# blubs/OpenGLRaytracer

Measured on AMD Instinct MI355X. Metric: primary Mrays/s at 1920×1080; achieved HBM GB/s vs peak; 1/2/4/8-GPU scaling, higher is better.
Workload: dtype f32

## Files before the change

include/rt.h:

```cpp
#ifndef OPENGLRAYTRACER_AMD_RT_H
#define OPENGLRAYTRACER_AMD_RT_H

#include <stddef.h>
#include <stdint.h>

#ifdef __cplusplus
extern "C" {
#endif

#define RT_OK 0
#define RT_ERR_INVALID (-1)
#define RT_ERR_HIP (-2)
#define RT_ERR_NOMEM (-3)
#define RT_ERR_UNSUPPORTED (-4)
#define RT_ERR_NO_DEVICE (-5)

#define RT_MAX_DEPTH 9

typedef struct rt_material {
    float ambient[4];
    float diffuse[4];
    float specular[4];
    float shininess;
    float emissive[4];
// ... 132 lines not shown

typedef struct rt_multi rt_multi;
#define RT_MULTI_RCCL 0
#define RT_MULTI_COPY 1
int rt_multi_create(int n_gpus, rt_context *const *ctxs, int transport, rt_multi **out);
void rt_multi_destroy(rt_multi *m);
int rt_render_multi(rt_multi *m, const rt_scene *const *scenes, const rt_camera *cam, float time, int width,
                    int height, int max_depth, int block_rows, float *out, int out_is_device);
int rt_render_multi_view(rt_multi *m, const rt_scene *const *scenes, const rt_view *view, int width, int height,
                         int max_depth, int block_rows, float *out, int out_is_device);
int rt_multi_last_ms(rt_multi *m, float *kernel_ms, float *gather_ms, float *assemble_ms);

#define RT_OPT_CULLING 1
#define RT_OPT_TIMING 2
#define RT_OPT_OUTPUT 3
#define RT_OUTPUT_RGBA32F 0
#define RT_OUTPUT_RGBA8 1
#define RT_OUTPUT_RGB32F 2
#define RT_OPT_FRAME_CONSTS 4
#define RT_OPT_ORIGIN_LISTS 7
#define RT_OPT_SCENE_SHAPES 8
#define RT_OPT_LAUNCH_SHAPES 9
#define RT_OPT_PERSISTENT0 10
int rt_context_set(rt_context *ctx, int option, int value);

int rt_last_kernel_ms(rt_context *ctx, float *ms);

int rt_pack_rgba8(const float *rgba32f, size_t n_pixels, uint8_t *out_rgba8);

int rt_write_ppm(const char *path, const float *rgba32f, int width, int height);
int rt_write_pfm(const char *path, const float *rgba32f, int width, int height);

const char *rt_last_error(void);
const char *rt_version(void);

#ifdef __cplusplus
}
#endif
#endif
```

openglraytracer_amd/__init__.py:

```python
import ctypes as C
import os

import numpy as np

from .abi import (RT_MAX_DEPTH, RT_OK, Camera, Light, Material, Object)
from . import abi

_HERE = os.path.dirname(os.path.abspath(__file__))
LIB_PATH = os.path.join(_HERE, "libopenglraytracer_amd.so")
_lib = None


class RTError(RuntimeError):
    def __init__(self, code, msg):
        super().__init__("rt error %d: %s" % (code, msg))
        self.code = code


class View(C.Structure):
    _fields_ = [("unprojection", C.c_float * 16), ("origin", C.c_float * 3)]


def lib():
    global _lib
# ... 218 lines not shown
        return self._h

    def set_culling(self, on):
        _check(lib().rt_context_set(self._h, abi.RT_OPT_CULLING, 1 if on else 0))

    def set_timing(self, on):
        _check(lib().rt_context_set(self._h, abi.RT_OPT_TIMING, 1 if on else 0))

    def set_host_frame_consts(self, on):
        _check(lib().rt_context_set(self._h, abi.RT_OPT_FRAME_CONSTS, 1 if on else 0))

    def set_origin_lists(self, on):
        _check(lib().rt_context_set(self._h, abi.RT_OPT_ORIGIN_LISTS, 1 if on else 0))

    def set_scene_shapes(self, on):
        _check(lib().rt_context_set(self._h, abi.RT_OPT_SCENE_SHAPES, 1 if on else 0))

    def set_launch_shapes(self, on):
        _check(lib().rt_context_set(self._h, abi.RT_OPT_LAUNCH_SHAPES, 1 if on else 0))

    def set_persistent0(self, value):
        _check(lib().rt_context_set(self._h, abi.RT_OPT_PERSISTENT0, int(value)))

    def set_output(self, fmt):
        _check(lib().rt_context_set(self._h, abi.RT_OPT_OUTPUT, fmt))
        self.output = fmt

    def last_kernel_ms(self):
        ms = C.c_float()
        _check(lib().rt_last_kernel_ms(self._h, C.byref(ms)))
        return ms.value


class Scene:

    def __init__(self, ctx, objects, materials=None, lights=None):
        materials = materials if materials is not None else reference_materials()
        lights = lights if lights is not None else reference_lights()
        objs = (Object * max(len(objects), 1))(*objects)
        mats = (Material * len(materials))(*materials)
        lts = (Light * max(len(lights), 1))(*lights)
        self._h = C.c_void_p()
        _check(lib().rt_scene_create(ctx.handle, objs, len(objects), mats, len(materials), lts,
                                     len(lights), C.byref(self._h)))
        self.ctx = ctx

# ... 219 lines not shown
```

openglraytracer_amd/abi.py:

```python
import ctypes as C

import numpy as np

RT_OK = 0
RT_ERR_INVALID = -1
RT_ERR_HIP = -2
RT_ERR_NOMEM = -3
RT_ERR_UNSUPPORTED = -4
RT_ERR_NO_DEVICE = -5
RT_MAX_DEPTH = 9
RT_MAX_OBJECTS = 1024
RT_MAX_LIGHTS = 16
RT_MAX_MATERIALS = 256
RT_OPT_CULLING = 1
RT_OPT_TIMING = 2
RT_OPT_OUTPUT = 3
RT_OPT_FRAME_CONSTS = 4
RT_OPT_ORIGIN_LISTS = 7
RT_OPT_SCENE_SHAPES = 8
RT_OPT_LAUNCH_SHAPES = 9
RT_OPT_PERSISTENT0 = 10
RT_OUTPUT_RGBA32F = 0
RT_OUTPUT_RGBA8 = 1
RT_OUTPUT_RGB32F = 2
RT_MAX_BATCH = 256
RT_MULTI_RCCL = 0
RT_MULTI_COPY = 1
RT_ANIM_NONE = 0
RT_ANIM_RATE = 1
RT_ANIM_RATE_OFFSET = 2
RT_ANIM_SIN = 3
RT_ANIM_SIN_OFFSET = 4

MATERIAL1, MATERIAL2, RED_GLASS, GREEN_GLASS, BLUE_GLASS, MIRROR, WALL = range(7)
MATERIAL_NAMES = ["material1", "material2", "red_glass_material", "green_glass_material",
                  "blue_glass_material", "mirror_material", "wall_material"]

F3 = C.c_float * 3
F4 = C.c_float * 4


class Material(C.Structure):
    _fields_ = [("ambient", F4), ("diffuse", F4), ("specular", F4), ("shininess", C.c_float),
                ("emissive", F4), ("reflectivity", C.c_float), ("transparency", C.c_float),
# ... 37 lines not shown
```

openglraytracer_amd/csrc/rt_api.cpp:

```cpp
#include <hip/hip_runtime.h>

#include <algorithm>
#include <climits>
#include <cmath>
#include <cstdio>
#include <cstring>
#include <new>
#include <string>
#include <type_traits>
#include <vector>

#include "build_id.h"
#include "rt_anim.h"
#include "rt_internal.h"

namespace rtamd {

namespace {
thread_local std::string g_error;
}

void set_error(const std::string &msg) { g_error = msg; }

int hip_fail(const char *what, hipError_t e) {
// ... 20 lines not shown
        set_error("null context or scene");
        return RT_ERR_INVALID;
    }
    if (scene->device != ctx->device) {
        set_error("scene was created on another device");
        return RT_ERR_INVALID;
    }
    if (width <= 0 || height <= 0 || width > 65536 || height > 65536) {
        set_error("bad frame size");
        return RT_ERR_INVALID;
    }
    if (max_depth < 0 || max_depth > RT_MAX_DEPTH) {
        set_error("max_depth " + std::to_string(max_depth) + " outside [0, " + std::to_string(RT_MAX_DEPTH) + "]");
        return RT_ERR_UNSUPPORTED;
    }
    return RT_OK;
}

bool fill_view(const rt_context *ctx, const rt_view &view, int width, int height, FrameView &v) {
    v = FrameView{};
    v.cull = (view_projection(view, v.proj) && ctx->culling) ? 1 : 0;
    std::memcpy(v.unproj, view.unprojection, sizeof v.unproj);
    std::memcpy(v.origin, view.origin, sizeof v.origin);
    return camera_short_divisions(v.unproj, width, height);
}

LaunchParams base_params(const rt_context *ctx, const rt_scene *scene, const rt_view *views, int n_views,
                         int width, int height, LaunchHost &h) {
    LaunchParams p{};
    p.n_views = n_views;
    p.cam_short = 1;
    h = LaunchHost{};
    h.shape_cull = ctx->scene_shapes;
    h.shape_launch = ctx->launch_shapes;
    h.persistent0 = ctx->persistent0;
    h.n_cu = ctx->n_cu;
    for (int k = 0; k < n_views; ++k) {
        if (!fill_view(ctx, views[k], width, height, p.view[k])) p.cam_short = 0;
        if (!p.view[k].cull) h.shape_cull = 0;
    }
    p.width = width;
    p.height = height;
    const DeviceScene &d = scene->dev;
    h.scene_room = d.room;
    p.scene = d.blob;
    p.layout = d.layout;
    if (!ctx->origin_lists) p.layout.off_olist = -1;
    p.out_format = ctx->output;
    if (ctx->host_consts) {
        const float4 *blobs[kMaxViews];
        for (int k = 0; k < n_views; ++k) blobs[k] = scene->host.empty() ? nullptr : scene->host.data();
        host_frame_setup(p, blobs);
    }
    return p;
}

int launch(rt_context *ctx, LaunchParams &p, const LaunchHost &h, int max_depth, hipStream_t stream) {
    const unsigned slot = ctx->sched_next % kSchedSlots;
// ... 187 lines not shown
        h.shape_cull = f[21];
        p.layout.off_dmask = f[22] > 0 ? 0 : -1;
        p.layout.dmask_bytes = f[22];
        p.layout.dmask_n = kShapeMaskTexels;
    }
    h.shape_launch = f[1];
    p.width = f[2];
    p.height = f[3];
    p.row_begin = f[4];
    p.n_rows = f[5];
    p.block_rows = f[6];
    p.n_shards = f[7];
    p.shard = f[8];
    p.out_format = f[9];
    p.n_frame_consts = f[10];
    p.cam_short = f[11];
    p.slice_begin = f[12];
    p.slice_rows = f[13];
    p.spp = f[14];
    return launch_shape(p, h, f[0], resident);
}
int rt_debug_launch_shape(const int32_t *f) { return rt_debug_launch_shape_n(f, 15); }
int rt_debug_last_queued(const rt_context *ctx) { return ctx ? (ctx->last_queued ? 1 : 0) : RT_ERR_INVALID; }
int rt_debug_last_scene_shape(const rt_context *ctx) { return ctx ? ctx->last_shape : RT_ERR_INVALID; }
int rt_debug_persistent_chunk(int c, int total, int waves, int32_t *out) {
    if (!out || c < 0 || total < 0 || total >= (1 << 30) || waves <= 0) return RT_ERR_INVALID;
    const ChunkRange r = persistent_chunk(c, total, waves);
    out[0] = r.t;
    out[1] = r.t_end;
    return RT_OK;
}
int rt_debug_persistent_queue(int g, int waves, int32_t *out) {
    if (!out || g < 0 || waves <= 0 || g >= waves) return RT_ERR_INVALID;
    out[0] = persistent_queue(g);
    out[1] = persistent_queue_waves(out[0], waves);
    out[2] = persistent_first_chunk(g);
    return RT_OK;
}
const char *rt_version(void) { return "openglraytracer_amd 0.3 (gfx950, " RT_BUILD_ID ")"; }

int rt_create(int device, rt_context **out) {
    if (!out) { set_error("rt_create: null out"); return RT_ERR_INVALID; }
    *out = nullptr;
    int n = 0;
    hipError_t e = hipGetDeviceCount(&n);
    if (e != hipSuccess || n <= 0) {
        set_error("rt_create: no HIP device");
// ... 472 lines not shown
    LaunchHost h;
    LaunchParams p = base_params(ctx, scene, view, 1, width, height, h);
    p.row_begin = row_begin;
    p.n_rows = row_end - row_begin;
    p.spp = spp;
    p.sample0 = sample_offset;
    p.seed = seed;
    p.jitter = jitter ? 1 : 0;
    p.out = reinterpret_cast<float4 *>(accum_device);
    hipStream_t stream = hip_stream ? static_cast<hipStream_t>(hip_stream) : ctx->stream;
    if ((rc = launch_scene(ctx, scene, p, h, max_depth, stream)) != RT_OK) return rc;
    return finish_call(hip_stream, stream);
}

int rt_context_set(rt_context *ctx, int option, int value) {
    if (!ctx) { set_error("rt_context_set: null context"); return RT_ERR_INVALID; }
    switch (option) {
        case RT_OPT_CULLING: ctx->culling = value ? 1 : 0; return RT_OK;
        case RT_OPT_TIMING: ctx->timing = value ? 1 : 0; return RT_OK;
        case RT_OPT_FRAME_CONSTS: ctx->host_consts = value ? 1 : 0; return RT_OK;
        case RT_OPT_ORIGIN_LISTS: ctx->origin_lists = value ? 1 : 0; return RT_OK;
        case RT_OPT_SCENE_SHAPES: ctx->scene_shapes = value ? 1 : 0; return RT_OK;
        case RT_OPT_LAUNCH_SHAPES: ctx->launch_shapes = value ? 1 : 0; return RT_OK;
        case RT_OPT_PERSISTENT0:
            if (value < 0 || (value > 1 && value < 8)) {
                set_error("rt_context_set: RT_OPT_PERSISTENT0 takes 0, 1 or a work-group cap of at least 8");
                return RT_ERR_INVALID;
            }
            ctx->persistent0 = value;
            return RT_OK;
        case RT_OPT_OUTPUT:
            if (value != RT_OUTPUT_RGBA32F && value != RT_OUTPUT_RGBA8 && value != RT_OUTPUT_RGB32F) {
                set_error("rt_context_set: unknown output format " + std::to_string(value));
                return RT_ERR_INVALID;
            }
            ctx->output = value;
            return RT_OK;
        default: set_error("rt_context_set: unknown option " + std::to_string(option)); return RT_ERR_INVALID;
    }
}

int rt_last_kernel_ms(rt_context *ctx, float *ms) {
    if (!ctx || !ms || !ctx->timed) {
        set_error("rt_last_kernel_ms: nothing timed yet");
        return RT_ERR_INVALID;
    }
// ... 256 lines not shown
```

openglraytracer_amd/csrc/rt_internal.h:

```cpp
#pragma once

#include <hip/hip_runtime.h>

#include <cstddef>
#include <cstdint>
#include <memory>
#include <string>
#include <vector>

#include "../../include/rt.h"

namespace rtamd {

struct SphereRec {
    float cx, cy, cz, rr;
};
struct SphereMeta {
    int32_t obj_index;
    int32_t material;
    float radius;
    int32_t pad;
};

struct BoxRec {
// ... 49 lines not shown
#define RT_OLIST_FROM 33
#endif
constexpr int kOListMinSpheres = RT_OLIST_FROM;
constexpr float kOListBoundUnit = 1.0f / 256.0f;
struct BvhNode {
    float lo[3];
    int32_t skip;
    float hi[3];
    int32_t leaf;
};
static_assert(sizeof(BvhNode) == 32, "BvhNode layout");
constexpr int kBvhOctants = 8;

struct LightRec {
    float pos[3];
    float dead;
};

struct FrameView {
    float unproj[16];
    float proj[16];
    float origin[3];
    int32_t cull;
    const void *blob;
};
constexpr int kMaxViews = 8;
constexpr int kBatchSlots = 4;
constexpr int kMaxFrameConsts = 272;
constexpr int kMaxViewConsts = 256;
constexpr size_t kMaxLds = 160 * 1024;

struct SceneLayout {
    int32_t off_spheres, off_smeta, off_boxes, off_mats, off_lights, off_lightmat;
    int32_t off_bvh, n_bvh;
    int32_t off_blink;
    int32_t off_cone;
    int32_t off_dmask, dmask_n;
    int32_t dmask_bytes;
    int32_t off_gmask, gmask_words;
    int32_t off_glist;
    int32_t blob_units;
    int32_t off_olist;
    int32_t dmask_box;
    int32_t off_bplane;
    int32_t n_spheres, n_boxes, n_mats, n_lights;
};

struct LaunchParams {
    FrameView view[kMaxViews];
    int32_t n_views;
    int32_t width, height;
    int32_t row_begin, n_rows;
    int32_t block_rows, n_shards, shard;
    const void *scene;
    float4 *out;
    int32_t spp, sample0, jitter;
    uint32_t seed;
    SceneLayout layout;
    int32_t *sched;
    int32_t out_format;
    int32_t n_frame_consts;
    int32_t cam_short;
    int32_t slice_begin, slice_rows;
    const FrameView *views_dev;
    const float4 *consts_dev;
    float4 frame_consts[kMaxFrameConsts];
};
static_assert(sizeof(LaunchParams) == 5776, "kernel argument block: the hidden arguments' offsets");
static_assert(offsetof(LaunchParams, layout) % 16 == 0, "the layout's offsets: aligned scalar loads (see above)");
static_assert(offsetof(LaunchParams, frame_consts) + sizeof(LaunchParams::frame_consts) == sizeof(LaunchParams),
              "kernarg_probe reads the last record: nothing the kernels read lies behind it");
static_assert(sizeof(LaunchParams) <= 6144, "kernel argument block");
struct LaunchHost {
    int32_t shape_cull;
    int32_t scene_room;
    int32_t shape_launch;
    int32_t persistent0;
    int32_t n_cu;
};
constexpr int kShapeMaskBytes = 15;
constexpr int kShapeMaskTexels = 12;
constexpr int kShapeRoom = 16;
constexpr int kShapeWide = 32;
int scene_shape(const SceneLayout &L, const LaunchHost &h, int max_depth);
constexpr int kLaunchPlain = 1;
constexpr int kLaunchPersistent = 2;
int launch_shape(const LaunchParams &p, const LaunchHost &h, int max_depth, int resident = 0);
#ifndef RT_CHUNK0
#define RT_CHUNK0 16
#endif
constexpr int kChunk0 = RT_CHUNK0;
static_assert(kChunk0 >= 2 && kChunk0 <= 32 && (kChunk0 & (kChunk0 - 1)) == 0, "bulk chunk: a power of two, 2..32");
struct ChunkRange {
    int t, t_end;
};
__host__ __device__ inline ChunkRange persistent_chunk(int c, int total, int waves) {
    int start = 0;
#pragma unroll
    for (int s = kChunk0; s >= 2; s >>= 1) {
        const int left = (total - start) / s - waves;
        const int n = left > 0 ? left : 0;
        if (c < n) return {start + c * s, start + c * s + s};
        c -= n;
        start += n * s;
    }
    return c < total - start ? ChunkRange{start + c, start + c + 1} : ChunkRange{total, total};
// ... 58 lines not shown
int ensure_origin_lists(rt_context *ctx, const rt_scene *scene, int max_depth);
int note_scene_use(const rt_scene *scene, hipStream_t stream, std::shared_ptr<UseEvent> *shared = nullptr);
int launch_scene(rt_context *ctx, const rt_scene *scene, LaunchParams &p, const LaunchHost &h, int max_depth,
                 hipStream_t stream);
inline size_t surface_bytes(int fmt) { return fmt == RT_OUTPUT_RGBA8 ? 4 : (fmt == RT_OUTPUT_RGB32F ? 12 : 16); }

}

struct rt_context {
    int device = 0;
    hipStream_t stream = nullptr;
    hipEvent_t ev0 = nullptr, ev1 = nullptr;
    float4 *staging = nullptr;
    size_t staging_px = 0;
    bool timed = false;
    int culling = 1;
    int timing = 1;
    int output = RT_OUTPUT_RGBA32F;
    int host_consts = 1;
    int origin_lists = 1;
    int scene_shapes = 1;
    int launch_shapes = 1;
    int persistent0 = 1;
    void *batch_dev[rtamd::kBatchSlots] = {};
    void *batch_host[rtamd::kBatchSlots] = {};
    hipEvent_t batch_done[rtamd::kBatchSlots] = {};
    bool batch_used[rtamd::kBatchSlots] = {};
    unsigned batch_next = 0;
    int n_cu = 0;
    int32_t *sched = nullptr;
    unsigned sched_next = 0;
    hipEvent_t sched_done[rtamd::kSchedSlots] = {};
    bool sched_used[rtamd::kSchedSlots] = {};
    bool last_queued = false;
    int last_shape = 0;
    std::vector<struct rt_scene *> scenes;
};

struct rt_scene {
    int device = 0;
    rtamd::DeviceScene dev;
    std::vector<float4> host;
    int32_t capacity_units = 0;
    rt_context *ctx = nullptr;
    static constexpr int kMaxUseStreams = 8;
    using Event = rtamd::UseEvent;
// ... 9 lines not shown
```

openglraytracer_amd/csrc/rt_kernel.hip:

```cpp
#include <hip/hip_runtime.h>

#include <algorithm>
#include <climits>
#include <cstdint>
#include <string>

#include "rt_internal.h"

namespace rtamd {
namespace {

constexpr int kWavesX = 2, kWavesY = 2;
constexpr int kTileX = 8 * kWavesX, kTileY = 8 * kWavesY;
constexpr int kThreads = 64 * kWavesX * kWavesY;

struct v3 {
    float x, y, z;
};
__device__ __forceinline__ v3 mk(float x, float y, float z) { return {x, y, z}; }
__device__ __forceinline__ v3 add(v3 a, v3 b) { return {a.x + b.x, a.y + b.y, a.z + b.z}; }
__device__ __forceinline__ v3 sub(v3 a, v3 b) { return {a.x - b.x, a.y - b.y, a.z - b.z}; }
__device__ __forceinline__ v3 muls(v3 a, float s) { return {a.x * s, a.y * s, a.z * s}; }
__device__ __forceinline__ v3 sel(bool c, v3 a, v3 b) { return {c ? a.x : b.x, c ? a.y : b.y, c ? a.z : b.z}; }
__device__ __forceinline__ float dot(v3 a, v3 b) { return a.x * b.x + (a.y * b.y + a.z * b.z); }

#ifdef RT_FAST_MATH
#define RT_FAST_DIV
#define RT_FAST_RSQ
// ... 1309 lines not shown
__device__ __forceinline__ Pixel wave_pixel(const LaunchParams &p, int wx, int wy) {
    const int lane = threadIdx.x & 63;
    Pixel px;
    px.x = wx * 8 + (lane & 7);
    if constexpr ((kLaunch & kLaunchPlain) != 0) {
        px.local_row = wy * 8 + (lane >> 3);
        px.active = px.x < p.width && px.local_row < p.height;
        px.y = px.active ? px.local_row : wy * 8;
        return px;
    }
    px.local_row = p.slice_begin + wy * 8 + (lane >> 3);
    px.active = px.x < p.width && px.local_row < p.slice_begin + p.slice_rows;
    px.y = output_row(p, px.active ? px.local_row : p.slice_begin + wy * 8);
    return px;
}

template <int kLaunch = 0>
__device__ __forceinline__ Ray camera_ray(const LaunchParams &p, const FrameView &V, int x, int y, float jx,
                                          float jy) {
    constexpr bool kPlain = (kLaunch & kLaunchPlain) != 0;
    const int hw = p.width / 2, hh = p.height / 2;
    const float *M = V.unproj;
    const float nx = static_cast<float>(x - hw) + jx, ny = static_cast<float>(y - hh) + jy;
    float vx, vy;
    if (kPlain || (hw > 0 && hh > 0)) {
        vx = div_r(nx, rcp_refined(static_cast<float>(hw)));
        vy = div_r(ny, rcp_refined(static_cast<float>(hh)));
    } else {
        vx = nx / static_cast<float>(hw);
        vy = ny / static_cast<float>(hh);
    }
    float ws[4], we[4];
#pragma unroll
    for (int k = 0; k < 4; ++k) {
        ws[k] = M[k] * vx + M[4 + k] * vy + M[8 + k] * 0.5f + M[12 + k] * 1.0f;
        we[k] = M[k] * vx + M[4 + k] * vy + M[8 + k] * 1.0f + M[12 + k] * 1.0f;
    }
    v3 s3, e3;
    if (kPlain || p.cam_short) {
        const Rcp rs3 = rcp_refined(ws[3]), re3 = rcp_refined(we[3]);
        s3 = mk(div_r(ws[0], rs3), div_r(ws[1], rs3), div_r(ws[2], rs3));
        e3 = mk(div_r(we[0], re3), div_r(we[1], re3), div_r(we[2], re3));
    } else {
        s3 = mk(fdiv(ws[0], ws[3]), fdiv(ws[1], ws[3]), fdiv(ws[2], ws[3]));
        e3 = mk(fdiv(we[0], we[3]), fdiv(we[1], we[3]), fdiv(we[2], we[3]));
    }
    Ray ray;
    ray.start = mk(V.origin[0], V.origin[1], V.origin[2]);
    ray.dir = normalize(sub(e3, s3));
    return ray;
}


template <int kDepth, bool kAccum, int kShape, int kLaunch = 0>
__device__ __forceinline__ void render_wave_tile(const LaunchParams &p, Scene S, const FrameView &V, int wx, int wy,
                                                 int z, const Pixel &px, const Ray &pre, bool have_pre) {
    S.cull = V.cull;
    S.room = 0;
// ... 91 lines not shown
    asm volatile("" : "+s"(a));
    return *(const LaunchParams *)a;
}
__device__ __forceinline__ float4 *persistent_slot(const LaunchParams &p, float4 *lds) {
    return lds + p.layout.blob_units + __builtin_amdgcn_readfirstlane(threadIdx.x >> 6) * p.n_frame_consts;
}
__device__ __forceinline__ void persistent_refill(const LaunchParams &p, float4 *lds, int z) {
    float4 *const slot = persistent_slot(p, lds);
    RT_PHASE_CLOCK(refill_t0);
    __builtin_amdgcn_fence(__ATOMIC_RELEASE, "wavefront");
    __builtin_amdgcn_wave_barrier();
    int lane = threadIdx.x & 63;
    asm volatile("" : "+v"(lane));
    for (int i = lane; i < p.n_frame_consts; i += 64) slot[i] = p.consts_dev[z * p.n_frame_consts + i];
    __builtin_amdgcn_fence(__ATOMIC_ACQUIRE, "wavefront");
    __builtin_amdgcn_wave_barrier();
    RT_PHASE_SPAN(10, 12, refill_t0);
}
template <int kShape, int kLaunch>
__device__ __forceinline__ void persistent_tile(const LaunchParams &p, float4 *lds, int z, int wx, int wy) {
    const float4 *blob = static_cast<const float4 *>(p.scene);
    float4 *const slot = persistent_slot(p, lds);
    const SceneLayout &L = p.layout;
    Scene S;
    S.sph = lds + L.off_spheres;
    S.smeta = reinterpret_cast<const int4 *>(lds + L.off_smeta);
    S.sph_cam = slot;
    S.sph_px = reinterpret_cast<const int4 *>(slot + L.n_spheres);
    S.box = reinterpret_cast<const BoxRec *>(lds + L.off_boxes);
    S.box_cam = slot + 2 * L.n_spheres;
    S.mat = reinterpret_cast<const MatRec *>(lds + L.off_mats);
    S.light = reinterpret_cast<const LightRec *>(lds + L.off_lights);
    S.lm = reinterpret_cast<const LightMatRec *>(lds + L.off_lightmat);
    S.bvh = lds + L.off_bvh;
    S.blink = reinterpret_cast<const uint32_t *>(lds + L.off_blink);
    S.cone = nullptr;
    S.dmask = reinterpret_cast<const char *>(lds + L.off_dmask);
    S.dmask_n = kShapeMaskTexels;
    S.dmask_bytes = kShape & kShapeMaskBytes;
    S.dmask_box = L.dmask_box;
    S.cbplane = L.off_bplane >= 0 ? (const __attribute__((address_space(4))) float4 *)(blob + L.off_bplane) : nullptr;
    S.gmask = nullptr;
    S.gwords = 0;
    S.glist = nullptr;
    S.olist = nullptr;
    S.cbox = (const __attribute__((address_space(4))) BoxRec *)(blob + L.off_boxes);
    S.clight = (const __attribute__((address_space(4))) LightRec *)(blob + L.off_lights);
#ifdef RT_UNIFORM_MAT
    S.cmat = (const __attribute__((address_space(4))) MatRec *)(blob + L.off_mats);
    S.clm = (const __attribute__((address_space(4))) LightMatRec *)(blob + L.off_lightmat);
#endif
    S.nbvh = 0;
    S.ns = L.n_spheres;
    S.nb = L.n_boxes;
    S.nl = L.n_lights;
    S.nm = L.n_mats;
    const FrameView V = cload((const __attribute__((address_space(4))) FrameView *)(p.views_dev) + z);
    const Ray none{mk(0.0f, 0.0f, 0.0f), mk(0.0f, 0.0f, 0.0f)};
    render_wave_tile<0, false, kShape, kLaunch>(p, S, V, wx, wy, z, wave_pixel<kLaunch>(p, wx, wy), none, false);
}
template <int kShape, int kLaunch>
__device__ __forceinline__ void render_persistent0(float4 *lds) {
    static_assert((kLaunch & kLaunchPlain) != 0 && (kShape & kShapeMaskBytes) != 0, "plain shaped launches");
    __builtin_amdgcn_s_setprio(1);
    RT_PHASE(0);
#ifdef RT_PHASE_TRACE
    if (RT_PHASE_LANE0) {
        RT_PHASE_SLOT(8) = __builtin_amdgcn_s_getreg((31 << 11) | 4) | (unsigned long long)__builtin_amdgcn_s_getreg((31 << 11) | 20) << 32;
    }
#endif
    {
        const LaunchParams &p = launch_args();
        const float4 *blob = static_cast<const float4 *>(p.scene);
// ... 273 lines not shown
    const void *fn = reinterpret_cast<const void *>(&render_kernel<kDepth, kAccum, kDev, kShape, kLaunch>);
    dim3 grid((p.width + kTileX - 1) / kTileX, (p.slice_rows + kTileY - 1) / kTileY, p.n_views);
    const int wave_tiles = ((p.width + 7) / 8) * ((p.slice_rows + 7) / 8) * p.n_views;
    const int resident = h.n_cu > 0 ? groups_per_cu(fn, lds) * h.n_cu : 0;
    bool one_scene = p.n_views <= kMaxViews;
    for (int k = 0; k < p.n_views && one_scene; ++k) one_scene = p.view[k].blob == nullptr;
    if (kQueuedDepth(kDepth) && p.sched && wave_tiles > resident * (kThreads / 64) &&
        resident * (kThreads / 64) >= kQueues &&
        (p.n_views == 1 || (one_scene && queued_views_for(fn, p.layout, kLean) >= p.n_views))) {
        grid = dim3(resident, 1, 1);
        lds = queued_lds_bytes(p.layout, kLean, p.n_views);
    } else {
        p.sched = nullptr;
    }
    hipLaunchKernelGGL((render_kernel<kDepth, kAccum, kDev, kShape, kLaunch>), grid, dim3(kThreads), lds, stream, p);
    return hipGetLastError();
}

size_t persistent_lds_bytes(const LaunchParams &p) {
    return (static_cast<size_t>(p.layout.blob_units) + static_cast<size_t>(kThreads / 64) * p.n_frame_consts) * sizeof(float4);
}

template <bool kAccum, bool kDev, int kShape>
hipError_t launch_shaped0(LaunchParams &p, const LaunchHost &h, hipStream_t stream) {
    if constexpr (!kAccum) {
        if ((launch_shape(p, h, 0) & kLaunchPlain) != 0) {
            if constexpr (kDev) {
                constexpr int kPersistent = kLaunchPlain | kLaunchPersistent;
                const size_t lds = persistent_lds_bytes(p);
                if (h.persistent0 > 0 && p.sched && lds <= kMaxLds && h.n_cu > 0) {
                    const void *fn = reinterpret_cast<const void *>(&render_kernel<0, false, true, kShape, kPersistent>);
                    const int groups = persistent_groups(p, h, groups_per_cu(fn, lds) * h.n_cu);
                    if (groups > 0) {
                        hipLaunchKernelGGL((render_kernel<0, false, true, kShape, kPersistent>), dim3(groups),
                                           dim3(kThreads), lds, stream, p);
                        return hipGetLastError();
                    }
                }
            }
            return launch_kernel<0, false, kDev, kShape, kLaunchPlain>(p, h, stream);
        }
    }
    return launch_kernel<0, kAccum, kDev, kShape>(p, h, stream);
}
template <bool kAccum, bool kDev>
hipError_t launch_depth0(LaunchParams &p, const LaunchHost &h, hipStream_t stream) {
    switch (scene_shape(p.layout, h, 0)) {
        case 2: return launch_shaped0<kAccum, kDev, 2>(p, h, stream);
        case 4: return launch_shaped0<kAccum, kDev, 4>(p, h, stream);
        case 8: return launch_shaped0<kAccum, kDev, 8>(p, h, stream);
        case 2 | kShapeRoom: return launch_shaped0<kAccum, kDev, 2 | kShapeRoom>(p, h, stream);
        case 4 | kShapeRoom: return launch_shaped0<kAccum, kDev, 4 | kShapeRoom>(p, h, stream);
        case 8 | kShapeRoom: return launch_shaped0<kAccum, kDev, 8 | kShapeRoom>(p, h, stream);
        default: return launch_kernel<0, kAccum, kDev, 0>(p, h, stream);
    }
}

template <int kDepth>
hipError_t launch_deep(LaunchParams &p, const LaunchHost &h, hipStream_t stream) {
    switch (scene_shape(p.layout, h, kDepth)) {
        case kShapeWide: return launch_kernel<kDepth, false, false, kShapeWide>(p, h, stream);
        case kShapeWide | kShapeRoom: return launch_kernel<kDepth, false, false, kShapeWide | kShapeRoom>(p, h, stream);
        default: return launch_kernel<kDepth, false, false, 0>(p, h, stream);
    }
}

template <int kDepth>
hipError_t launch_depth(LaunchParams &p, const LaunchHost &h, hipStream_t stream) {
    if (p.views_dev) {
        if constexpr (kDepth == 0) {
            if (p.spp == 0) return launch_depth0<false, true>(p, h, stream);
        } else if constexpr (kDepth == 1) {
            if (p.spp == 0) return launch_kernel<kDepth, false, true>(p, h, stream);
        }
        return hipErrorInvalidValue;
    }
    if constexpr (kDepth == 0) return p.spp > 0 ? launch_depth0<true, false>(p, h, stream) : launch_depth0<false, false>(p, h, stream);
    if constexpr (kDepth >= 2) {
        if (p.spp == 0) return launch_deep<kDepth>(p, h, stream);
    }
    return p.spp > 0 ? launch_kernel<kDepth, true>(p, h, stream) : launch_kernel<kDepth, false>(p, h, stream);
}

}

int scene_shape(const SceneLayout &L, const LaunchHost &h, int max_depth) {
    if (!h.shape_cull) return 0;
    const int box = L.n_boxes == 1 && h.scene_room ? kShapeRoom : 0;
    if (max_depth == 0) {
        if (L.off_dmask < 0 || (L.dmask_bytes != 2 && L.dmask_bytes != 4 && L.dmask_bytes != 8) ||
            L.dmask_n != kShapeMaskTexels)
            return 0;
        return L.dmask_bytes | box;
    }
    if (max_depth >= 2) {
        if (L.off_gmask < 0 || L.off_glist < 0 || L.off_olist < 0) return 0;
        return kShapeWide | box;
    }
    return 0;
}

int persistent_groups(const LaunchParams &p, const LaunchHost &h, int resident) {
#if defined(RT_STATS) || defined(RT_CYCLES)
    return 0;
#endif
    if (h.persistent0 <= 0 || (launch_shape(p, h, 0) & kLaunchPlain) == 0 || scene_shape(p.layout, h, 0) == 0) return 0;
    if (!p.views_dev || !p.consts_dev || p.n_views <= kMaxViews || !p.sched) return 0;
    const bool forced = h.persistent0 >= 8;
    const int groups = forced && h.persistent0 < resident ? h.persistent0 : resident;
    const long long waves = static_cast<long long>(groups) * (kThreads / 64);
    const long long tiles = static_cast<long long>((p.width + 7) / 8) * ((p.height + 7) / 8) * p.n_views;
    if (waves < kQueues || tiles >= (1ll << 30)) return 0;
    if (!forced && tiles < kPersistentMinTilesPerWave * waves) return 0;
    return groups;
}

// ... 74 lines not shown
        (void)hipFree(d);
    }
    if (e != hipSuccess) {
        set_error(std::string("rt_create: kernel argument probe: ") + hipGetErrorString(e));
        return RT_ERR_HIP;
    }
    if (h[0].x != 1.5f || h[0].y != -2.25f || h[0].z != 3.125f || h[0].w != 4096.0f ||
        __builtin_bit_cast(uint32_t, h[1].x) != 0x5a5au || __builtin_bit_cast(uint32_t, h[1].y) != 0x3c3cu) {
        set_error("rt_create: this HIP runtime does not pass a " + std::to_string(sizeof(LaunchParams)) +
                  "-byte kernel argument block intact");
        return RT_ERR_UNSUPPORTED;
    }
    return RT_OK;
}

hipError_t allow_large_lds(size_t bytes) {
#define RT_KFN(d) reinterpret_cast<const void *>(&render_kernel<d, false>), \
                  reinterpret_cast<const void *>(&render_kernel<d, true>)
#define RT_SHAPES(k) reinterpret_cast<const void *>(&render_kernel<0, false, false, k>), \
                     reinterpret_cast<const void *>(&render_kernel<0, true, false, k>),  \
                     reinterpret_cast<const void *>(&render_kernel<0, false, true, k>),  \
                     reinterpret_cast<const void *>(&render_kernel<0, false, false, k, kLaunchPlain>), \
                     reinterpret_cast<const void *>(&render_kernel<0, false, true, k, kLaunchPlain>), \
                     reinterpret_cast<const void *>(&render_kernel<0, false, true, k, kLaunchPlain | kLaunchPersistent>)
#define RT_WIDE(d) reinterpret_cast<const void *>(&render_kernel<d, false, false, kShapeWide>), \
                   reinterpret_cast<const void *>(&render_kernel<d, false, false, kShapeWide | kShapeRoom>)
    const void *fns[] = {RT_KFN(0), RT_KFN(1), RT_KFN(2), RT_KFN(3), RT_KFN(4),
                         RT_KFN(5), RT_KFN(6), RT_KFN(7), RT_KFN(8), RT_KFN(9),
                         reinterpret_cast<const void *>(&render_kernel<0, false, true>),
                         reinterpret_cast<const void *>(&render_kernel<1, false, true>),
                         RT_SHAPES(2), RT_SHAPES(4), RT_SHAPES(8),
                         RT_SHAPES(2 | kShapeRoom), RT_SHAPES(4 | kShapeRoom), RT_SHAPES(8 | kShapeRoom),
                         RT_WIDE(2), RT_WIDE(3), RT_WIDE(4), RT_WIDE(5), RT_WIDE(6), RT_WIDE(7), RT_WIDE(8), RT_WIDE(9)};
#undef RT_KFN
#undef RT_SHAPES
#undef RT_WIDE
    for (const void *f : fns)
        (void)hipFuncSetAttribute(f, hipFuncAttributeMaxDynamicSharedMemorySize, static_cast<int>(bytes));
    (void)hipGetLastError();
    return hipSuccess;
}

}

#ifdef RT_STATS
extern "C" int rt_debug_stats(unsigned long long *dst, int clear) {
    if (hipMemcpyFromSymbol(dst, HIP_SYMBOL(rtamd::rt_stats), sizeof(rtamd::rt_stats), 0, hipMemcpyDeviceToHost) !=
// ... 42 lines not shown
```

openglraytracer_amd/csrc/rt_scene.cpp:

```cpp
#include <algorithm>
#include <cmath>
#include <cstring>
#include <map>
#include <memory>
#include <mutex>
#include <new>
#include <system_error>
#include <thread>
#include <vector>

#include "rt_anim.h"
#include "rt_internal.h"

using namespace rtamd;

namespace {

constexpr float kPi = 3.14159265358f;
constexpr float kDegToRad = kPi / 180.0f;

struct M4 {
    double m[4][4];
};

// ... 1011 lines not shown
        for (int i = 0; i < n_objs; ++i)
            for (int k = 0; k < 3; ++k)
                finite = finite && std::isfinite(objs[i].position[k]) && std::isfinite(objs[i].box_mins[k]) &&
                         std::isfinite(objs[i].box_maxs[k]) && std::isfinite(objs[i].radius);
        bplane.assign(boxes.size() * static_cast<size_t>(n_lights), no_plane());
        for (size_t b = 0; b < boxes.size() && finite; ++b)
            for (int j = 0; j < n_lights; ++j)
                bplane[b * n_lights + j] = box_light_plane(boxes[b], lights[j].position, extent);
        lay.off_bplane = off;
        off += units(bplane.size() * sizeof(float4));
    }
    lay.off_bvh = off;     off += units(bvh.size() * sizeof(BvhNode));
    lay.off_blink = off;   off += units(blink.size() * sizeof(uint32_t));
    const size_t per_frame = sph.size() * 32 + boxes.size() * 16;
    int n_live = 0;
    for (int j = 0; j < n_lights; ++j) n_live += lrec[j].dead == 0.0f;
    std::vector<uint64_t> dmask;
    lay.off_dmask = -1;
    lay.dmask_n = 0;
    const bool box_bits = boxes.size() >= 2;
    const size_t mask_bits = sph.size() + (box_bits ? boxes.size() : 0);
    lay.dmask_box = 0;
    lay.dmask_bytes = 4;
    if (!sph.empty() && mask_bits <= static_cast<size_t>(kMaskMaxSpheres) && n_live > 0) {
        lay.dmask_bytes = mask_bits <= 16 ? 2 : (mask_bits <= 32 ? 4 : 8);
#ifndef RT_DMASK_MAXN
#define RT_DMASK_MAXN 12
#endif
        for (int n : {32, 24, 16, 12, 8}) {
            if (n > RT_DMASK_MAXN) continue;
            const size_t bytes = static_cast<size_t>(n_live) * 6 * n * n * lay.dmask_bytes;
            if ((static_cast<size_t>(off) + units(bytes)) * 16 + per_frame <= kMaskLdsBudget) {
                lay.dmask_n = n;
                break;
            }
        }
    }
    std::vector<char> dmask_bytes;
    if (lay.dmask_n > 0) {
        if (box_bits) {
            std::vector<SphereRec> bsph(sph);
            std::vector<SphereMeta> bmeta(smeta);
            for (size_t b = 0; b < boxes.size(); ++b) {
                bsph.push_back({ball[b].x, ball[b].y, ball[b].z, 0.0f});
                bmeta.push_back({boxes[b].obj_index, boxes[b].material, ball[b].w, 0});
            }
            build_direction_masks(bsph, bmeta, lights, lrec, lay.dmask_n, dmask);
            lay.dmask_box = 1;
        } else {
            build_direction_masks(sph, smeta, lights, lrec, lay.dmask_n, dmask);
        }
        lay.off_dmask = off;
        dmask_bytes.resize(dmask.size() * lay.dmask_bytes);
        for (size_t i = 0; i < dmask.size(); ++i)
            std::memcpy(dmask_bytes.data() + i * lay.dmask_bytes, &dmask[i], lay.dmask_bytes);
        off += units(dmask_bytes.size());
        cones.clear();
    }
    const size_t with_cones = (static_cast<size_t>(off) + units(cones.size() * sizeof(ShadowCone))) * 16 + per_frame;
    if (lay.dmask_n == 0 && with_cones <= kConeLdsBudget) {
        lay.off_cone = off;
        off += units(cones.size() * sizeof(ShadowCone));
    } else {
        lay.off_cone = -1;
        cones.clear();
    }
    lay.n_bvh = static_cast<int32_t>(bvh.size());
    lay.blob_units = off;
    std::vector<uint64_t> gmask;
    std::vector<uint8_t> glist;
    lay.off_gmask = -1;
    lay.off_glist = -1;
    lay.gmask_words = 0;
#ifndef RT_GMASK_FROM
#define RT_GMASK_FROM 32
#endif
    if (sph.size() > static_cast<size_t>(RT_GMASK_FROM) &&
        sph.size() <= static_cast<size_t>(kGMaskMaxSpheres) && n_live > 0) {
        lay.gmask_words = static_cast<int32_t>((sph.size() + 63) / 64);
        build_direction_masks(sph, smeta, lights, lrec, kGMaskTexels, gmask, lay.gmask_words);
// ... 448 lines not shown
```

Baseline: 80090.

## Use compile-time fixed scene blob layout and host-precomputed view terms

```diff
diff --git a/include/rt.h b/include/rt.h
--- a/include/rt.h
+++ b/include/rt.h
@@ -178,6 +178,7 @@
 #define RT_OPT_SCENE_SHAPES 8
 #define RT_OPT_LAUNCH_SHAPES 9
 #define RT_OPT_PERSISTENT0 10
+#define RT_OPT_FIXED_LAYOUT 11
 int rt_context_set(rt_context *ctx, int option, int value);
 
 int rt_last_kernel_ms(rt_context *ctx, float *ms);
diff --git a/openglraytracer_amd/__init__.py b/openglraytracer_amd/__init__.py
--- a/openglraytracer_amd/__init__.py
+++ b/openglraytracer_amd/__init__.py
@@ -264,6 +264,9 @@
     def set_persistent0(self, value):
         _check(lib().rt_context_set(self._h, abi.RT_OPT_PERSISTENT0, int(value)))
 
+    def set_fixed_layout(self, on):
+        _check(lib().rt_context_set(self._h, abi.RT_OPT_FIXED_LAYOUT, 1 if on else 0))
+
     def set_output(self, fmt):
         _check(lib().rt_context_set(self._h, abi.RT_OPT_OUTPUT, fmt))
         self.output = fmt
diff --git a/openglraytracer_amd/abi.py b/openglraytracer_amd/abi.py
--- a/openglraytracer_amd/abi.py
+++ b/openglraytracer_amd/abi.py
@@ -20,6 +20,7 @@
 RT_OPT_SCENE_SHAPES = 8
 RT_OPT_LAUNCH_SHAPES = 9
 RT_OPT_PERSISTENT0 = 10
+RT_OPT_FIXED_LAYOUT = 11
 RT_OUTPUT_RGBA32F = 0
 RT_OUTPUT_RGBA8 = 1
 RT_OUTPUT_RGB32F = 2
diff --git a/openglraytracer_amd/csrc/rt_api.cpp b/openglraytracer_amd/csrc/rt_api.cpp
--- a/openglraytracer_amd/csrc/rt_api.cpp
+++ b/openglraytracer_amd/csrc/rt_api.cpp
@@ -66,6 +66,9 @@
     v.cull = (view_projection(view, v.proj) && ctx->culling) ? 1 : 0;
     std::memcpy(v.unproj, view.unprojection, sizeof v.unproj);
     std::memcpy(v.origin, view.origin, sizeof v.origin);
+    for (int k = 0; k < 4; ++k) v.unproj_half[k] = v.unproj[8 + k] * 0.5f;
+    v.rcp_hw = 1.0f / static_cast<float>(width / 2);
+    v.rcp_hh = 1.0f / static_cast<float>(height / 2);
     return camera_short_divisions(v.unproj, width, height);
 }
 
@@ -78,6 +81,7 @@
     h.shape_cull = ctx->scene_shapes;
     h.shape_launch = ctx->launch_shapes;
     h.persistent0 = ctx->persistent0;
+    h.fixed_layout = ctx->fixed_layout;
     h.n_cu = ctx->n_cu;
     for (int k = 0; k < n_views; ++k) {
         if (!fill_view(ctx, views[k], width, height, p.view[k])) p.cam_short = 0;
@@ -311,7 +315,34 @@
 }
 int rt_debug_launch_shape(const int32_t *f) { return rt_debug_launch_shape_n(f, 15); }
 int rt_debug_last_queued(const rt_context *ctx) { return ctx ? (ctx->last_queued ? 1 : 0) : RT_ERR_INVALID; }
-int rt_debug_last_scene_shape(const rt_context *ctx) { return ctx ? ctx->last_shape : RT_ERR_INVALID; }
+int rt_debug_last_scene_shape(const rt_context *ctx) { return ctx ? (ctx->last_shape & ~kShapeFixed) : RT_ERR_INVALID; }
+int rt_debug_last_fixed_layout(const rt_context *ctx) {
+    return ctx ? ((ctx->last_shape & kShapeFixed) != 0 ? 1 : 0) : RT_ERR_INVALID;
+}
+int rt_debug_fixed_layout(const rt_object *objs, int n_objs, const rt_material *mats, int n_mats,
+                          const rt_light *lights, int n_lights, int32_t *out) {
+    if (!out) return RT_ERR_INVALID;
+    std::vector<float4> blob;
+    DeviceScene ds;
+    const int rc = build_scene(objs, n_objs, mats, n_mats, lights, n_lights, blob, ds);
+    if (rc != RT_OK) return rc;
+    const SceneLayout &L = ds.layout;
+    LaunchHost h{};
+    h.shape_cull = 1;
+    h.scene_room = ds.room;
+    h.fixed_layout = 1;
+    const FixedLayout f = fixed_layout(L.n_boxes == 1);
+    out[0] = layout_is_fixed(L) ? 1 : 0;
+    out[1] = scene_shape(L, h, 0);
+    h.fixed_layout = 0;
+    out[2] = scene_shape(L, h, 0);
+    out[3] = L.dmask_n;
+    out[4] = L.blob_units;
+    const int32_t o[7] = {f.off_spheres, f.off_smeta(L.n_spheres), f.off_boxes, f.off_mats, f.off_lights, f.off_lightmat,
+                          f.off_dmask(L.n_spheres)};
+    std::memcpy(out + 5, o, sizeof o);
+    return RT_OK;
+}
 int rt_debug_persistent_chunk(int c, int total, int waves, int32_t *out) {
     if (!out || c < 0 || total < 0 || total >= (1 << 30) || waves <= 0) return RT_ERR_INVALID;
     const ChunkRange r = persistent_chunk(c, total, waves);
@@ -830,6 +861,7 @@
         case RT_OPT_ORIGIN_LISTS: ctx->origin_lists = value ? 1 : 0; return RT_OK;
         case RT_OPT_SCENE_SHAPES: ctx->scene_shapes = value ? 1 : 0; return RT_OK;
         case RT_OPT_LAUNCH_SHAPES: ctx->launch_shapes = value ? 1 : 0; return RT_OK;
+        case RT_OPT_FIXED_LAYOUT: ctx->fixed_layout = value ? 1 : 0; return RT_OK;
         case RT_OPT_PERSISTENT0:
             if (value < 0 || (value > 1 && value < 8)) {
                 set_error("rt_context_set: RT_OPT_PERSISTENT0 takes 0, 1 or a work-group cap of at least 8");
diff --git a/openglraytracer_amd/csrc/rt_internal.h b/openglraytracer_amd/csrc/rt_internal.h
--- a/openglraytracer_amd/csrc/rt_internal.h
+++ b/openglraytracer_amd/csrc/rt_internal.h
@@ -95,8 +95,15 @@
     float proj[16];
     float origin[3];
     int32_t cull;
+    float unproj_half[4];
+    float rcp_hw, rcp_hh;
     const void *blob;
 };
+static_assert(sizeof(FrameView) == 176 && offsetof(FrameView, unproj_half) % 16 == 0, "FrameView: whole 16-B units");
+#ifndef RT_HOST_VIEW_TERMS
+#define RT_HOST_VIEW_TERMS 1
+#endif
+constexpr bool kHostViewTerms = RT_HOST_VIEW_TERMS != 0;
 constexpr int kMaxViews = 8;
 constexpr int kBatchSlots = 4;
 constexpr int kMaxFrameConsts = 272;
@@ -139,7 +146,7 @@
     const float4 *consts_dev;
     float4 frame_consts[kMaxFrameConsts];
 };
-static_assert(sizeof(LaunchParams) == 5776, "kernel argument block: the hidden arguments' offsets");
+static_assert(sizeof(LaunchParams) == 5968, "kernel argument block: the hidden arguments' offsets");
 static_assert(offsetof(LaunchParams, layout) % 16 == 0, "the layout's offsets: aligned scalar loads (see above)");
 static_assert(offsetof(LaunchParams, frame_consts) + sizeof(LaunchParams::frame_consts) == sizeof(LaunchParams),
               "kernarg_probe reads the last record: nothing the kernels read lies behind it");
@@ -149,12 +156,42 @@
     int32_t scene_room;
     int32_t shape_launch;
     int32_t persistent0;
+    int32_t fixed_layout;
     int32_t n_cu;
 };
 constexpr int kShapeMaskBytes = 15;
 constexpr int kShapeMaskTexels = 12;
 constexpr int kShapeRoom = 16;
 constexpr int kShapeWide = 32;
+constexpr int kShapeFixed = 64;
+constexpr int kFixedMaxLights = 3, kFixedMaxMats = 7, kFixedMaxBoxes = 4;
+struct FixedLayout {
+    int32_t off_boxes, off_mats, off_lights, off_lightmat, off_spheres;
+    __host__ __device__ constexpr int32_t off_smeta(int n) const { return off_spheres + n; }
+    __host__ __device__ constexpr int32_t off_dmask(int n) const { return off_spheres + 2 * n; }
+};
+static_assert(sizeof(SphereRec) == 16 && sizeof(SphereMeta) == 16, "a unit per sphere and table");
+__host__ __device__ constexpr FixedLayout fixed_layout(bool one_box) {
+    FixedLayout f{};
+    f.off_boxes = 0;
+    f.off_mats = f.off_boxes + (one_box ? 1 : kFixedMaxBoxes) * static_cast<int>(sizeof(BoxRec) / 16);
+    f.off_lights = f.off_mats + kFixedMaxMats * static_cast<int>(sizeof(MatRec) / 16);
+    f.off_lightmat = f.off_lights + kFixedMaxLights * static_cast<int>(sizeof(LightRec) / 16);
+    f.off_spheres = f.off_lightmat + kFixedMaxMats * kFixedMaxLights * static_cast<int>(sizeof(LightMatRec) / 16);
+    return f;
+}
+inline bool fixed_counts(int n_spheres, int n_boxes, int n_mats, int n_lights) {
+    return n_spheres >= 1 && n_boxes >= 1 && n_boxes <= kFixedMaxBoxes && n_lights >= 1 &&
+           n_lights <= kFixedMaxLights && n_mats >= 1 && n_mats <= kFixedMaxMats &&
+           n_spheres + (n_boxes >= 2 ? n_boxes : 0) <= kMaskMaxSpheres;
+}
+inline bool layout_is_fixed(const SceneLayout &L) {
+    if (L.off_dmask < 0 || !fixed_counts(L.n_spheres, L.n_boxes, L.n_mats, L.n_lights)) return false;
+    const FixedLayout f = fixed_layout(L.n_boxes == 1);
+    return L.off_boxes == f.off_boxes && L.off_mats == f.off_mats && L.off_lights == f.off_lights &&
+           L.off_lightmat == f.off_lightmat && L.off_spheres == f.off_spheres &&
+           L.off_smeta == f.off_smeta(L.n_spheres) && L.off_dmask == f.off_dmask(L.n_spheres);
+}
 int scene_shape(const SceneLayout &L, const LaunchHost &h, int max_depth);
 constexpr int kLaunchPlain = 1;
 constexpr int kLaunchPersistent = 2;
@@ -259,6 +296,7 @@
     int scene_shapes = 1;
     int launch_shapes = 1;
     int persistent0 = 1;
+    int fixed_layout = 1;
     void *batch_dev[rtamd::kBatchSlots] = {};
     void *batch_host[rtamd::kBatchSlots] = {};
     hipEvent_t batch_done[rtamd::kBatchSlots] = {};
diff --git a/openglraytracer_amd/csrc/rt_kernel.hip b/openglraytracer_amd/csrc/rt_kernel.hip
--- a/openglraytracer_amd/csrc/rt_kernel.hip
+++ b/openglraytracer_amd/csrc/rt_kernel.hip
@@ -4,6 +4,7 @@
 #include <climits>
 #include <cstdint>
 #include <string>
+#include <type_traits>
 
 #include "rt_internal.h"
 
@@ -1359,8 +1360,12 @@
     const int hw = p.width / 2, hh = p.height / 2;
     const float *M = V.unproj;
     const float nx = static_cast<float>(x - hw) + jx, ny = static_cast<float>(y - hh) + jy;
+    constexpr bool kHostTerms = kPlain && kHostViewTerms;
     float vx, vy;
-    if (kPlain || (hw > 0 && hh > 0)) {
+    if (kHostTerms) {
+        vx = div_r(nx, Rcp{static_cast<float>(hw), V.rcp_hw});
+        vy = div_r(ny, Rcp{static_cast<float>(hh), V.rcp_hh});
+    } else if (kPlain || (hw > 0 && hh > 0)) {
         vx = div_r(nx, rcp_refined(static_cast<float>(hw)));
         vy = div_r(ny, rcp_refined(static_cast<float>(hh)));
     } else {
@@ -1370,7 +1375,7 @@
     float ws[4], we[4];
 #pragma unroll
     for (int k = 0; k < 4; ++k) {
-        ws[k] = M[k] * vx + M[4 + k] * vy + M[8 + k] * 0.5f + M[12 + k] * 1.0f;
+        ws[k] = M[k] * vx + M[4 + k] * vy + (kHostTerms ? V.unproj_half[k] : M[8 + k] * 0.5f) + M[12 + k] * 1.0f;
         we[k] = M[k] * vx + M[4 + k] * vy + M[8 + k] * 1.0f + M[12 + k] * 1.0f;
     }
     v3 s3, e3;
@@ -1508,20 +1513,22 @@
     const float4 *blob = static_cast<const float4 *>(p.scene);
     float4 *const slot = persistent_slot(p, lds);
     const SceneLayout &L = p.layout;
+    constexpr bool kFixed = (kShape & kShapeFixed) != 0;
+    constexpr FixedLayout F = fixed_layout((kShape & kShapeRoom) != 0);
     Scene S;
-    S.sph = lds + L.off_spheres;
-    S.smeta = reinterpret_cast<const int4 *>(lds + L.off_smeta);
+    S.sph = lds + (kFixed ? F.off_spheres : L.off_spheres);
+    S.smeta = reinterpret_cast<const int4 *>(lds + (kFixed ? F.off_smeta(L.n_spheres) : L.off_smeta));
     S.sph_cam = slot;
     S.sph_px = reinterpret_cast<const int4 *>(slot + L.n_spheres);
-    S.box = reinterpret_cast<const BoxRec *>(lds + L.off_boxes);
+    S.box = reinterpret_cast<const BoxRec *>(lds + (kFixed ? F.off_boxes : L.off_boxes));
     S.box_cam = slot + 2 * L.n_spheres;
-    S.mat = reinterpret_cast<const MatRec *>(lds + L.off_mats);
-    S.light = reinterpret_cast<const LightRec *>(lds + L.off_lights);
-    S.lm = reinterpret_cast<const LightMatRec *>(lds + L.off_lightmat);
+    S.mat = reinterpret_cast<const MatRec *>(lds + (kFixed ? F.off_mats : L.off_mats));
+    S.light = reinterpret_cast<const LightRec *>(lds + (kFixed ? F.off_lights : L.off_lights));
+    S.lm = reinterpret_cast<const LightMatRec *>(lds + (kFixed ? F.off_lightmat : L.off_lightmat));
     S.bvh = lds + L.off_bvh;
     S.blink = reinterpret_cast<const uint32_t *>(lds + L.off_blink);
     S.cone = nullptr;
-    S.dmask = reinterpret_cast<const char *>(lds + L.off_dmask);
+    S.dmask = reinterpret_cast<const char *>(lds + (kFixed ? F.off_dmask(L.n_spheres) : L.off_dmask));
     S.dmask_n = kShapeMaskTexels;
     S.dmask_bytes = kShape & kShapeMaskBytes;
     S.dmask_box = L.dmask_box;
@@ -1530,11 +1537,11 @@
     S.gwords = 0;
     S.glist = nullptr;
     S.olist = nullptr;
-    S.cbox = (const __attribute__((address_space(4))) BoxRec *)(blob + L.off_boxes);
-    S.clight = (const __attribute__((address_space(4))) LightRec *)(blob + L.off_lights);
+    S.cbox = (const __attribute__((address_space(4))) BoxRec *)(blob + (kFixed ? F.off_boxes : L.off_boxes));
+    S.clight = (const __attribute__((address_space(4))) LightRec *)(blob + (kFixed ? F.off_lights : L.off_lights));
 #ifdef RT_UNIFORM_MAT
-    S.cmat = (const __attribute__((address_space(4))) MatRec *)(blob + L.off_mats);
-    S.clm = (const __attribute__((address_space(4))) LightMatRec *)(blob + L.off_lightmat);
+    S.cmat = (const __attribute__((address_space(4))) MatRec *)(blob + (kFixed ? F.off_mats : L.off_mats));
+    S.clm = (const __attribute__((address_space(4))) LightMatRec *)(blob + (kFixed ? F.off_lightmat : L.off_lightmat));
 #endif
     S.nbvh = 0;
     S.ns = L.n_spheres;
@@ -1854,20 +1861,25 @@
 }
 
 template <bool kAccum, bool kDev, int kShape>
-hipError_t launch_shaped0(LaunchParams &p, const LaunchHost &h, hipStream_t stream) {
+hipError_t launch_shaped0(LaunchParams &p, const LaunchHost &h, hipStream_t stream, bool fixed) {
     if constexpr (!kAccum) {
         if ((launch_shape(p, h, 0) & kLaunchPlain) != 0) {
             if constexpr (kDev) {
                 constexpr int kPersistent = kLaunchPlain | kLaunchPersistent;
                 const size_t lds = persistent_lds_bytes(p);
                 if (h.persistent0 > 0 && p.sched && lds <= kMaxLds && h.n_cu > 0) {
-                    const void *fn = reinterpret_cast<const void *>(&render_kernel<0, false, true, kShape, kPersistent>);
-                    const int groups = persistent_groups(p, h, groups_per_cu(fn, lds) * h.n_cu);
-                    if (groups > 0) {
-                        hipLaunchKernelGGL((render_kernel<0, false, true, kShape, kPersistent>), dim3(groups),
-                                           dim3(kThreads), lds, stream, p);
-                        return hipGetLastError();
-                    }
+                    const auto run = [&](auto shape) {
+                        constexpr int kS = decltype(shape)::value;
+                        const void *fn = reinterpret_cast<const void *>(&render_kernel<0, false, true, kS, kPersistent>);
+                        const int groups = persistent_groups(p, h, groups_per_cu(fn, lds) * h.n_cu);
+                        if (groups > 0)
+                            hipLaunchKernelGGL((render_kernel<0, false, true, kS, kPersistent>), dim3(groups),
+                                               dim3(kThreads), lds, stream, p);
+                        return groups;
+                    };
+                    const int groups = fixed ? run(std::integral_constant<int, kShape | kShapeFixed>{})
+                                             : run(std::integral_constant<int, kShape>{});
+                    if (groups > 0) return hipGetLastError();
                 }
             }
             return launch_kernel<0, false, kDev, kShape, kLaunchPlain>(p, h, stream);
@@ -1877,13 +1889,15 @@
 }
 template <bool kAccum, bool kDev>
 hipError_t launch_depth0(LaunchParams &p, const LaunchHost &h, hipStream_t stream) {
-    switch (scene_shape(p.layout, h, 0)) {
-        case 2: return launch_shaped0<kAccum, kDev, 2>(p, h, stream);
-        case 4: return launch_shaped0<kAccum, kDev, 4>(p, h, stream);
-        case 8: return launch_shaped0<kAccum, kDev, 8>(p, h, stream);
-        case 2 | kShapeRoom: return launch_shaped0<kAccum, kDev, 2 | kShapeRoom>(p, h, stream);
-        case 4 | kShapeRoom: return launch_shaped0<kAccum, kDev, 4 | kShapeRoom>(p, h, stream);
-        case 8 | kShapeRoom: return launch_shaped0<kAccum, kDev, 8 | kShapeRoom>(p, h, stream);
+    const int shape = scene_shape(p.layout, h, 0);
+    const bool fixed = (shape & kShapeFixed) != 0;
+    switch (shape & ~kShapeFixed) {
+        case 2: return launch_shaped0<kAccum, kDev, 2>(p, h, stream, fixed);
+        case 4: return launch_shaped0<kAccum, kDev, 4>(p, h, stream, fixed);
+        case 8: return launch_shaped0<kAccum, kDev, 8>(p, h, stream, fixed);
+        case 2 | kShapeRoom: return launch_shaped0<kAccum, kDev, 2 | kShapeRoom>(p, h, stream, fixed);
+        case 4 | kShapeRoom: return launch_shaped0<kAccum, kDev, 4 | kShapeRoom>(p, h, stream, fixed);
+        case 8 | kShapeRoom: return launch_shaped0<kAccum, kDev, 8 | kShapeRoom>(p, h, stream, fixed);
         default: return launch_kernel<0, kAccum, kDev, 0>(p, h, stream);
     }
 }
@@ -1923,7 +1937,8 @@
         if (L.off_dmask < 0 || (L.dmask_bytes != 2 && L.dmask_bytes != 4 && L.dmask_bytes != 8) ||
             L.dmask_n != kShapeMaskTexels)
             return 0;
-        return L.dmask_bytes | box;
+        const bool fixed = h.fixed_layout && layout_is_fixed(L) && (box != 0) == (L.n_boxes == 1);
+        return L.dmask_bytes | box | (fixed ? kShapeFixed : 0);
     }
     if (max_depth >= 2) {
         if (L.off_gmask < 0 || L.off_glist < 0 || L.off_olist < 0) return 0;
@@ -2044,7 +2059,8 @@
                      reinterpret_cast<const void *>(&render_kernel<0, false, true, k>),  \
                      reinterpret_cast<const void *>(&render_kernel<0, false, false, k, kLaunchPlain>), \
                      reinterpret_cast<const void *>(&render_kernel<0, false, true, k, kLaunchPlain>), \
-                     reinterpret_cast<const void *>(&render_kernel<0, false, true, k, kLaunchPlain | kLaunchPersistent>)
+                     reinterpret_cast<const void *>(&render_kernel<0, false, true, k, kLaunchPlain | kLaunchPersistent>), \
+                     reinterpret_cast<const void *>(&render_kernel<0, false, true, k | kShapeFixed, kLaunchPlain | kLaunchPersistent>)
 #define RT_WIDE(d) reinterpret_cast<const void *>(&render_kernel<d, false, false, kShapeWide>), \
                    reinterpret_cast<const void *>(&render_kernel<d, false, false, kShapeWide | kShapeRoom>)
     const void *fns[] = {RT_KFN(0), RT_KFN(1), RT_KFN(2), RT_KFN(3), RT_KFN(4),
diff --git a/openglraytracer_amd/csrc/rt_scene.cpp b/openglraytracer_amd/csrc/rt_scene.cpp
--- a/openglraytracer_amd/csrc/rt_scene.cpp
+++ b/openglraytracer_amd/csrc/rt_scene.cpp
@@ -1057,17 +1057,34 @@
     const size_t mask_bits = sph.size() + (box_bits ? boxes.size() : 0);
     lay.dmask_box = 0;
     lay.dmask_bytes = 4;
+    bool fixed = false;
     if (!sph.empty() && mask_bits <= static_cast<size_t>(kMaskMaxSpheres) && n_live > 0) {
         lay.dmask_bytes = mask_bits <= 16 ? 2 : (mask_bits <= 32 ? 4 : 8);
 #ifndef RT_DMASK_MAXN
 #define RT_DMASK_MAXN 12
 #endif
-        for (int n : {32, 24, 16, 12, 8}) {
-            if (n > RT_DMASK_MAXN) continue;
-            const size_t bytes = static_cast<size_t>(n_live) * 6 * n * n * lay.dmask_bytes;
-            if ((static_cast<size_t>(off) + units(bytes)) * 16 + per_frame <= kMaskLdsBudget) {
-                lay.dmask_n = n;
-                break;
+        const auto texels = [&](int32_t head) {
+            for (int n : {32, 24, 16, 12, 8}) {
+                if (n > RT_DMASK_MAXN) continue;
+                const size_t bytes = static_cast<size_t>(n_live) * 6 * n * n * lay.dmask_bytes;
+                if ((static_cast<size_t>(head) + units(bytes)) * 16 + per_frame <= kMaskLdsBudget) return n;
+            }
+            return 0;
+        };
+        lay.dmask_n = texels(off);
+        if (lay.dmask_n > 0 && fixed_counts(static_cast<int>(sph.size()), static_cast<int>(boxes.size()), n_mats, n_lights)) {
+            const FixedLayout f = fixed_layout(boxes.size() == 1);
+            const int32_t n_sph = static_cast<int32_t>(sph.size());
+            const int32_t tail = off - lay.off_lightmat - units(lm.size() * sizeof(LightMatRec));
+            if (texels(f.off_dmask(n_sph) + tail) == lay.dmask_n) {
+                fixed = true;
+                lay.off_boxes = f.off_boxes;
+                lay.off_mats = f.off_mats;
+                lay.off_lights = f.off_lights;
+                lay.off_lightmat = f.off_lightmat;
+                lay.off_spheres = f.off_spheres;
+                lay.off_smeta = f.off_smeta(n_sph);
+                off = f.off_dmask(n_sph);
             }
         }
     }
@@ -1091,6 +1108,14 @@
             std::memcpy(dmask_bytes.data() + i * lay.dmask_bytes, &dmask[i], lay.dmask_bytes);
         off += units(dmask_bytes.size());
         cones.clear();
+    }
+    if (fixed) {
+        if (lay.off_bplane >= 0) {
+            lay.off_bplane = off;
+            off += units(bplane.size() * sizeof(float4));
+        }
+        lay.off_bvh = off;     off += units(bvh.size() * sizeof(BvhNode));
+        lay.off_blink = off;   off += units(blink.size() * sizeof(uint32_t));
     }
     const size_t with_cones = (static_cast<size_t>(off) + units(cones.size() * sizeof(ShadowCone))) * 16 + per_frame;
     if (lay.dmask_n == 0 && with_cones <= kConeLdsBudget) {
```

After: 81760 (median of 6 runs). 1.02x the previous value.
